# davrempe/contact-human-dynamics

Hardware: NVIDIA H100
Metric: optimised frames/sec (batched phys-optim) (higher is better)
Workload: dtype f64

## Files before the change

__graft_entry__.py:

```python
import os
import subprocess
import sys

ROOT = os.path.dirname(os.path.abspath(__file__))
if ROOT not in sys.path:
    sys.path.insert(0, ROOT)


def build() -> None:
    subprocess.check_call(["make", "-C", os.path.join(ROOT, "contact-human-dynamics_b200", "csrc")])
    subprocess.check_call(["make", "-C", os.path.join(ROOT, "oracle")])
    subprocess.check_call(["make", "-C", os.path.join(ROOT, "tests", "kkt")])
    import chd
    chd.phys.load_lib()


def smoke() -> None:
    import numpy as np
    import chd
    from oracle.phys import OracleProblem
    ps = chd.synth.make_batch(2, 120, 2, seed0=100)
    b = chd.phys.PhysBatch(ps, device=0)
    ev = b.eval("2.2")
    o = OracleProblem(ps[0])
    o.set_stage("2.2")
    n = o.n
    np.testing.assert_allclose(ev["cost"][0], o.cost(), rtol=1e-10)
    np.testing.assert_allclose(ev["grad"][0, :n], o.grad(), rtol=1e-9, atol=1e-9)
    out = b.solve()
    st = out["stage_status"]
    assert (st[[0, 1, 2, 3]] == 0).all() and ((st[4] == 0) | (st[5] == 0)).all(), st
    ref = o.solve()
    ids = {"1.1": 0, "1.2": 1, "2.1": 2, "2.2": 3, "3": 4, "4": 5}
    assert [s["status"] for s in ref["stages"]] == [int(st[ids[k], 0]) for k in ref["stage_ids"]]
    got = out["samples"][2, 0, :out["frames"][0]]
    exp = ref["durations"]
    np.testing.assert_allclose(got[:, :12], exp[:, :12], rtol=0, atol=1e-4)
    np.testing.assert_allclose(got[:, 12:18], exp[:, 12:18], rtol=0, atol=1e-2)
    np.testing.assert_array_equal(got[:, 18:], exp[:, 18:])
    print("smoke ok: launches=%d" % b.launch_count())


if __name__ == "__main__":
    build()
    if len(sys.argv) > 1 and sys.argv[1] == "smoke":
# ... 2 lines not shown
```

contact-human-dynamics_b200/csrc/chd_api.cu:

```cuda
#include <cuda_runtime.h>

#include <cstdio>
#include <cstdlib>
#include <cstring>
#include <vector>

#include "../../include/chd.h"
#include "chd_dev.h"

__global__ void chd_k_stage_begin(ChdDev D);
template <bool GLOBAL>
__global__ void chd_k_eval(ChdDev D);
__global__ void chd_k_init(ChdDev D);
__global__ void chd_k_kkt(ChdDev D);
__global__ void chd_k_kkt_gwin(ChdDev D);
__global__ void chd_k_kcopy(ChdDev D);
__global__ void chd_k_curv(ChdDev D);
__global__ void chd_k_asm(ChdDev D);
__global__ void chd_k_fp64_peak(int mode, int iters, double* sink);
__global__ void chd_k_hess_base(ChdDev D);
__global__ void chd_k_hess_dur(ChdDev D);
__global__ void chd_k_hess_zero(ChdDev D);
__global__ void chd_k_hess_fin(ChdDev D, int mode);
__global__ void chd_k_tables(ChdDev D);
__global__ void chd_k_clear_dyn(ChdDev D);
template <bool GLOBAL>
__global__ void chd_k_linesearch(ChdDev D);
__global__ void chd_k_sample(ChdDev D, double* out, int* frames_out);
__global__ void chd_k_snapshot(ChdDev D, int* frames_out);
__global__ void chd_k_sched_reset(ChdDev D);

#define CHD_CUDA(x)                                                                          \
  do {                                                                                       \
    cudaError_t e_ = (x);                                                                    \
    if (e_ != cudaSuccess) {                                                                 \
      fprintf(stderr, "libchd: CUDA error %s at %s:%d\n", cudaGetErrorString(e_), __FILE__, __LINE__); \
      return -100 - (int)e_;                                                                 \
    }                                                                                        \
  } while (0)

enum { KT_EVAL = 0, KT_KKT = 1, KT_LS = 2, KT_INIT = 3, KT_SAMPLE = 4, KT_N = 8 };

struct ChdIterForm {
  void (*eval)(ChdDev);
  void (*linesearch)(ChdDev);
  size_t smem_eval, smem_ls;
};
static ChdIterForm chd_iter_form(int n_max, int smem_optin) {
  const size_t red = CHD_THREADS * sizeof(double);
  if ((2 * (size_t)n_max + CHD_THREADS) * sizeof(double) + 1024 <= (size_t)smem_optin)
    return {chd_k_eval<false>, chd_k_linesearch<false>, 2 * (size_t)n_max * sizeof(double) + red,
            (size_t)n_max * sizeof(double) + red};
  return {chd_k_eval<true>, chd_k_linesearch<true>, red, red};
}

struct chd_phys_batch {
  ChdHostBatch hb;
  ChdDev D;
  std::vector<void*> allocs;
  cudaStream_t stream = nullptr, copy_stream = nullptr;
  cudaEvent_t ev_kkt = nullptr, ev_ls = nullptr, ev_copy = nullptr;
  int64_t launches = 0;
  int timing = 0;
  bool host_only = false;
  double kt_ms[KT_N] = {0};
  int64_t kt_n[KT_N] = {0};
  cudaEvent_t ev0 = nullptr, ev1 = nullptr;
  int* d_frames = nullptr;
  double* d_samples = nullptr;
  ChdIterForm iter = {};
  size_t smem_kkt = 0;
  int kcopy_blocks = 1;
  ChdIpm* h_ipm = nullptr;
  double* d_x0 = nullptr;
  int64_t h2d_bytes = 0;
  ChdStageDev* d_stages = nullptr;
  int sched_max_iter = 0;
  bool sched_has_dur = false;
  double *poly_T0 = nullptr, *poly_tend0 = nullptr, *phase_tend0 = nullptr;
  int* ent_col0 = nullptr;
};

namespace {

template <class T>
int dev_upload(chd_phys_batch* b, const std::vector<T>& v, const T** out) {
  void* p = nullptr;
  size_t bytes = std::max<size_t>(v.size(), 1) * sizeof(T);
  CHD_CUDA(cudaMallocAsync(&p, bytes, b->stream));
  b->allocs.push_back(p);
  if (!v.empty()) CHD_CUDA(cudaMemcpyAsync(p, v.data(), v.size() * sizeof(T), cudaMemcpyHostToDevice, b->stream));
  b->h2d_bytes += (int64_t)(v.size() * sizeof(T));
  *out = (const T*)p;
  return 0;
}
template <class T>
int dev_alloc(chd_phys_batch* b, size_t count, T** out) {
  void* p = nullptr;
  CHD_CUDA(cudaMallocAsync(&p, std::max<size_t>(count, 1) * sizeof(T), b->stream));
  CHD_CUDA(cudaMemsetAsync(p, 0, std::max<size_t>(count, 1) * sizeof(T), b->stream));
  b->allocs.push_back(p);
  *out = (T*)p;
  return 0;
}
// ... 22 lines not shown
      cudaEventRecord(b->ev1, b->stream);
      cudaEventSynchronize(b->ev1);
      float ms = 0;
      cudaEventElapsedTime(&ms, b->ev0, b->ev1);
      b->kt_ms[id] += ms;
    }
  }
};

void launch_eval(chd_phys_batch* b) {
  Timer t(b, KT_EVAL);
  b->iter.eval<<<b->hb.B, CHD_THREADS, b->iter.smem_eval, b->stream>>>(b->D);
}

int set_schedule(chd_phys_batch* b, const int* sched, int nsched, int override_stage, int override_max_iter) {
  ChdStageDev tab[6];
  for (int s = 0; s < 6; ++s) tab[s] = stage_dev(b->hb.stage[s], s);
  if (override_stage >= 0 && override_max_iter > 0) tab[override_stage].max_iter = override_max_iter;
  CHD_CUDA(cudaMemcpyAsync(b->d_stages, tab, sizeof(tab), cudaMemcpyHostToDevice, b->stream));
  b->D.stages = b->d_stages;
  b->D.nsched = nsched;
  for (int i = 0; i < nsched; ++i) b->D.sched[i] = sched[i];
  b->sched_max_iter = 0;
  b->sched_has_dur = false;
  for (int i = 0; i < nsched; ++i) b->sched_max_iter += tab[sched[i]].max_iter + 2, b->sched_has_dur |= sched[i] == CHD_STAGE_3;
  chd_k_sched_reset<<<(b->hb.B + 127) / 128, 128, 0, b->stream>>>(b->D);
  b->launches++;
  return 0;
}

int run_schedule(chd_phys_batch* b) {
  const int B = b->hb.B;
  const int check_every = 8;
  for (int it = 0; it <= b->sched_max_iter; ++it) {
    {
      Timer t(b, KT_INIT);
      chd_k_stage_begin<<<B, CHD_THREADS, 0, b->stream>>>(b->D);
    }
    launch_eval(b);
    {
      Timer t(b, KT_INIT);
      chd_k_init<<<B, CHD_THREADS, 0, b->stream>>>(b->D);
    }
    {
      Timer t(b, KT_INIT);
      chd_k_hess_zero<<<dim3(8, B), 256, 0, b->stream>>>(b->D);
      chd_k_hess_base<<<dim3(16, B), 256, 0, b->stream>>>(b->D);
      chd_k_hess_fin<<<B, 128, 0, b->stream>>>(b->D, 0);
      b->launches += 2;
    }
    CHD_CUDA(cudaStreamWaitEvent(b->stream, b->ev_copy, 0));
    chd_k_asm<<<dim3(8, B), 256, 0, b->stream>>>(b->D);
    b->launches++;
    {
      Timer t(b, KT_KKT);
      if (b->D.win_smem) chd_k_kkt<<<B, CHD_KKT_THREADS, b->smem_kkt, b->stream>>>(b->D);
      else chd_k_kkt_gwin<<<B, CHD_KKT_THREADS, b->smem_kkt, b->stream>>>(b->D);
    }
    CHD_CUDA(cudaEventRecord(b->ev_kkt, b->stream));
    CHD_CUDA(cudaStreamWaitEvent(b->copy_stream, b->ev_kkt, 0));
    chd_k_kcopy<<<dim3(b->kcopy_blocks, B), 256, 0, b->copy_stream>>>(b->D);
    b->launches++;
    {
      Timer t(b, KT_LS);
      b->iter.linesearch<<<B, CHD_THREADS, b->iter.smem_ls, b->stream>>>(b->D);
    }
    CHD_CUDA(cudaEventRecord(b->ev_ls, b->stream));
    CHD_CUDA(cudaStreamWaitEvent(b->copy_stream, b->ev_ls, 0));
    if (b->sched_has_dur) {
      chd_k_hess_dur<<<dim3(8, B), CHD_THREADS, 0, b->copy_stream>>>(b->D);
      chd_k_hess_fin<<<B, 128, 0, b->copy_stream>>>(b->D, 1);
      b->launches += 2;
    }
    chd_k_curv<<<dim3(8, B), 256, 0, b->copy_stream>>>(b->D);
    b->launches++;
    CHD_CUDA(cudaEventRecord(b->ev_copy, b->copy_stream));
    {
      Timer t(b, KT_SAMPLE);
      chd_k_snapshot<<<B, 128, 0, b->stream>>>(b->D, b->d_frames);
    }
    if ((it % check_every) == check_every - 1) {
      CHD_CUDA(cudaMemcpyAsync(b->h_ipm, b->D.ipm, B * sizeof(ChdIpm), cudaMemcpyDeviceToHost, b->stream));
      CHD_CUDA(cudaStreamSynchronize(b->stream));
      bool any = false;
      for (int i = 0; i < B; ++i) any |= (b->h_ipm[i].phase != CHD_PH_FINISHED);
      if (!any) break;
    }
  }
  CHD_CUDA(cudaMemcpyAsync(b->h_ipm, b->D.ipm, B * sizeof(ChdIpm), cudaMemcpyDeviceToHost, b->stream));
  CHD_CUDA(cudaStreamSynchronize(b->stream));
  CHD_CUDA(cudaStreamSynchronize(b->copy_stream));
  CHD_CUDA(cudaGetLastError());
  return 0;
}

}

extern "C" {

const char* chd_version(void) { return "libchd 0.1 (sm_90a)"; }

int chd_measure_fp64_peak(double* dfma_gflops, double* dmma_gflops) {
  int dev = 0, sms = 0;
  CHD_CUDA(cudaGetDevice(&dev));
  CHD_CUDA(cudaDeviceGetAttribute(&sms, cudaDevAttrMultiProcessorCount, dev));
  double* sink = nullptr;
  CHD_CUDA(cudaMalloc((void**)&sink, sizeof(double) * 1024));
  cudaEvent_t e0, e1;
  CHD_CUDA(cudaEventCreate(&e0));
  CHD_CUDA(cudaEventCreate(&e1));
  const int blocks = sms * 8, threads = 256, iters = 4096;
  for (int mode = 0; mode < 2; ++mode) {
    float best = 1e30f;
    for (int rep = 0; rep < 4; ++rep) {
      CHD_CUDA(cudaEventRecord(e0));
      chd_k_fp64_peak<<<blocks, threads>>>(mode, iters, sink);
      CHD_CUDA(cudaEventRecord(e1));
      CHD_CUDA(cudaEventSynchronize(e1));
      float ms = 0;
// ... 79 lines not shown
  AL(sc, mm) AL(dL, mm) AL(dU, mm) AL(s, mm) AL(y, mm) AL(zL, mm) AL(zU, mm) AL(ds, mm) AL(dy, mm) AL(dzL, mm) AL(dzU, mm)
  int dev = 0, sms = 0, smem_max = 0;
  CHD_CUDA(cudaGetDevice(&dev));
  CHD_CUDA(cudaDeviceGetAttribute(&sms, cudaDevAttrMultiProcessorCount, dev));
  CHD_CUDA(cudaDeviceGetAttribute(&smem_max, cudaDevAttrMaxSharedMemoryPerBlockOptin, dev));
  cudaFuncAttributes fa_kkt, fa_gwin;
  CHD_CUDA(cudaFuncGetAttributes(&fa_kkt, chd_k_kkt));
  CHD_CUDA(cudaFuncGetAttributes(&fa_gwin, chd_k_kkt_gwin));
  const ChdKktPlan P = chd_kkt_plan(hb.Na_max, hb.nb_max, hb.w_max, hb.w_fix_max, hb.n_max, fa_kkt.sharedSizeBytes,
                                    fa_gwin.sharedSizeBytes, (size_t)smem_max);
  D.win_smem = P.win_smem, D.nbc_max = P.nbc_max, D.Q = P.Q, D.Qfix = P.Qfix, D.nbt = P.nbt, D.win_tiles = P.win_tiles;
  D.pan_doubles = P.pan_doubles, D.kstride = P.kstride, D.scratch_stride = P.scratch_stride;
  b->smem_kkt = P.smem_bytes;
  b->kcopy_blocks = (int)std::min<size_t>(512, std::max<size_t>(std::max<size_t>(1, 4 * (size_t)sms / B), P.kstride * sizeof(double) / 131072));
  AL(cost, B * 2) AL(Kwork, B * P.kstride) AL(Kbase, B * P.kstride) AL(sol, B * (size_t)(hb.Na_max + hb.nb_max)) AL(ipm, B)
  AL(rhs0, B * (size_t)(hb.Na_max + hb.nb_max)) AL(rhs1, B * (size_t)(hb.Na_max + hb.nb_max))
  if (P.scratch_stride) AL(scratch, B * P.scratch_stride)
#undef AL
  if ((rc = dev_upload(b, hb.x0, (const double**)&b->d_x0))) return rc;
  CHD_CUDA(cudaMemcpyAsync(D.x, b->d_x0, nm * sizeof(double), cudaMemcpyDeviceToDevice, b->stream));
  b->iter = chd_iter_form(hb.n_max, smem_max);
  if (P.status == CHD_KKT_TOO_WIDE_COMPACT || P.status == CHD_KKT_TOO_WIDE_PAIRS) {
    fprintf(stderr, "libchd: band + border too wide for the %s (Q=%d nbt=%d)\n",
            P.status == CHD_KKT_TOO_WIDE_COMPACT ? "compacted update loop" : "pair tables", P.Q, P.nbt);
    return -5;
  }
  if (P.status == CHD_KKT_TOO_LARGE) {
    fprintf(stderr, "libchd: KKT band + border too large for the shared memory of the factorisation (n_max=%d)\n", hb.n_max);
    return -5;
  }
  CHD_CUDA(cudaFuncSetAttribute(b->iter.eval, cudaFuncAttributeMaxDynamicSharedMemorySize, (int)b->iter.smem_eval));
  CHD_CUDA(cudaFuncSetAttribute(P.win_smem ? chd_k_kkt : chd_k_kkt_gwin, cudaFuncAttributeMaxDynamicSharedMemorySize, (int)b->smem_kkt));
  CHD_CUDA(cudaFuncSetAttribute(b->iter.linesearch, cudaFuncAttributeMaxDynamicSharedMemorySize, (int)b->iter.smem_ls));
  const size_t stride = 6 + 7 * (size_t)hb.n_ee_max;
  CHD_CUDA(cudaMallocAsync((void**)&b->d_samples, B * hb.fo_max * stride * sizeof(double), b->stream));
  CHD_CUDA(cudaMallocAsync((void**)&b->d_frames, B * sizeof(int), b->stream));
  b->allocs.push_back(b->d_samples);
  b->allocs.push_back(b->d_frames);
  b->h_ipm = (ChdIpm*)std::malloc(B * sizeof(ChdIpm));
  if (!b->h_ipm) return -3;
  CHD_CUDA(cudaMallocAsync((void**)&b->d_stages, 6 * sizeof(ChdStageDev), b->stream));
  b->allocs.push_back(b->d_stages);
  if ((rc = dev_alloc(b, 3 * B * hb.fo_max * stride, &D.snapshots))) return rc;
  CHD_CUDA(cudaStreamSynchronize(b->stream));
  return 0;
}

void chd_phys_batch_destroy(chd_phys_batch* b) {
  if (!b) return;
  if (b->stream) {
    for (void* p : b->allocs) cudaFreeAsync(p, b->stream);
    cudaStreamSynchronize(b->stream);
  }
  std::free(b->h_ipm);
  if (b->ev0) cudaEventDestroy(b->ev0);
  if (b->ev1) cudaEventDestroy(b->ev1);
  if (b->ev_kkt) cudaEventDestroy(b->ev_kkt);
  if (b->ev_copy) cudaEventDestroy(b->ev_copy);
  if (b->ev_ls) cudaEventDestroy(b->ev_ls);
  if (b->copy_stream) cudaStreamDestroy(b->copy_stream);
  if (b->stream) cudaStreamDestroy(b->stream);
  delete b;
}

int chd_phys_get_dims(const chd_phys_batch* b, chd_phys_dims* d) {
  if (!b || !d) return -1;
// ... 231 lines not shown
```

contact-human-dynamics_b200/csrc/chd_kkt.cu:

```cuda
#include <cuda_runtime.h>

#include "chd_block.cuh"
#include "chd_eval.cuh"
#include "chd_kkt_tiles.cuh"

__device__ __forceinline__ void chd_hess_sample(const ChdCtx& c, const ChdKT& K, const int* vk, int s, const ChdSpl* P, const double* sign, int np,
                                                int deriv, double wgt, int lane, double* ws) {
  const bool tau = c.opt_dur && s >= 2 && deriv == 0;
  if (lane < 28) {
    const int pa = lane / 14, q = lane % 14;
    double v0 = 0.0, v1 = 0.0, v2 = 0.0;
    int ia = -1;
    if (pa < np) {
      if (q < 12) {
        const int va = P[pa].var[q];
        const double wa = sign[pa] * chd_slot_w(P[pa], deriv, q);
        if (va >= 0 && wa != 0.0) {
          ia = vk[va];
          v0 = q % 3 == 0 ? wa : 0.0, v1 = q % 3 == 1 ? wa : 0.0, v2 = q % 3 == 2 ? wa : 0.0;
        }
      } else if (tau) {
        ChdTau u;
        chd_spl_tau(c, s, s - 2, P[pa], u);
        const int var = q == 12 ? u.va : u.vb;
        const double* dv = q == 12 ? u.da : u.db;
        if (var >= 0) ia = vk[var], v0 = sign[pa] * dv[0], v1 = sign[pa] * dv[1], v2 = sign[pa] * dv[2];
      }
    }
    ws[lane * 4 + 0] = (double)ia, ws[lane * 4 + 1] = v0, ws[lane * 4 + 2] = v1, ws[lane * 4 + 3] = v2;
  }
  __syncwarp();
  const int ne = np * 14;
// ... 274 lines not shown
        if (ka < 0) continue;
        const double va = sc * Jv[ea];
        if (va == 0.0) continue;
        g_add(ka, -va * coef0, va * beta);
        for (int eb = e0; eb < e1; ++eb) {
          const int cb = ec[eb];
          if (cb < 0) continue;
          const int kb = vk[cb];
          if (kb < 0 || ka < kb) continue;
          const double vb = sc * Jv[eb];
          if (vb != 0.0) chd_kadd(K, ka, kb, Sig * va * vb);
        }
      }
    }
  }
}

struct ChdKktCtx {
  int b, tid, nt, lane, warp, nwarp;
  ChdIpm* I;
  ChdStageDev sg;
  const ChdSeq* h;
  int n, m, n_act, Qs, Q, nbt, nbp8, nbl, nbc, NBR, nbt_s;
  size_t ro, vo, n_even, xs_len, win_region;
  const int *rf, *vk, *rk, *ep, *ec;
  const double *Jv, *grad;
  ChdKT K;
  double *red, *cc, *ypan, *xpan, *dinv, *win, *bwin, *vecn, *xs, *xs2;
  double sf, mu, tau, delta_w;
  bool polish;
};

template <bool WS>
__device__ __forceinline__ void chd_kkt_ctx_init(const ChdDev& D, ChdIpm& I, ChdKktCtx& c) {
  extern __shared__ double sm[];
  const int b = blockIdx.x;
  c.b = b, c.I = &I;
  c.sg = D.stages[I.stage];
  const ChdSeq* h = c.h = D.seq + b;
  c.n = h->n, c.m = h->m, c.tid = threadIdx.x, c.nt = blockDim.x;
  c.lane = c.tid & 31, c.warp = c.tid >> 5, c.nwarp = c.nt >> 5;
  c.ro = (size_t)b * D.m_max, c.vo = (size_t)b * D.n_max;
  c.rf = D.rflag + c.ro;
  c.vk = D.var_kkt + c.vo;
  c.rk = D.row_kkt + c.ro;
  c.ep = D.ent_ptr + (size_t)b * (D.m_max + 1);
  c.ec = D.ent_col + (size_t)b * D.slots_max;
  c.Jv = D.Jv + (size_t)b * D.slots_max;
  c.grad = D.grad + c.vo;
  ChdKT& K = c.K;
  chd_kt_init(D, h, D.Kwork + (size_t)b * D.kstride, K);
  K.ovf = &I.band_ovf;
  if (!c.sg.opt_dur) K.q = D.Qfix - 1;
  c.n_act = c.sg.opt_dur ? c.n : c.n - h->n_dur;
  c.Qs = K.Q, c.Q = c.sg.opt_dur ? K.Q : D.Qfix, c.nbt = K.nbt, c.nbp8 = K.nbp8, c.nbl = c.sg.opt_dur ? h->nb : h->nb_fix, c.nbc = K.nbc;
  c.NBR = c.nbl, c.nbt_s = (c.nbl + 1 + 7) >> 3;
  c.n_even = (size_t)((D.n_max + 1) & ~1), c.xs_len = (size_t)(8 * D.nbc_max + c.nbp8);
  double* gs = WS ? nullptr : D.scratch + (size_t)b * D.scratch_stride;
  c.red = sm;
  c.cc = c.red + CHD_KKT_THREADS;
  c.ypan = c.cc + c.nbp8 * c.nbp8;
  c.xpan = c.ypan + (c.Q + c.nbt) * 64;
  c.dinv = c.ypan + D.pan_doubles;
  c.win_region = (size_t)D.win_tiles * 64 + (size_t)c.Qs * c.nbt * 64;
  c.win = WS ? c.dinv + 16 : gs + c.n_even + c.xs_len + 8 * (size_t)D.nbc_max;
  c.bwin = c.win + (size_t)D.win_tiles * 64;
  c.vecn = WS ? c.win + c.win_region - c.n_even : gs;
  c.xs = WS ? c.vecn - c.xs_len : c.vecn + c.n_even;
  c.xs2 = WS ? c.ypan : c.xs + c.xs_len;
  c.sf = I.sf;
}

__device__ __forceinline__ bool chd_kkt_errors(const ChdDev& D, ChdKktCtx& c, int& s_fail) {
  ChdIpm& I = *c.I;
  const int b = c.b, tid = c.tid, nt = c.nt, n = c.n, m = c.m, n_act = c.n_act;
  const size_t ro = c.ro, vo = c.vo;
  const int *rf = c.rf, *vk = c.vk, *ep = c.ep, *ec = c.ec;
  const double *Jv = c.Jv, *grad = c.grad, sf = c.sf;
  double* red = c.red;
  double mu = I.mu;
  const int* erow = D.ent_row + (size_t)b * D.slots_max;
  const int* cptr = D.col_ptr + (size_t)b * (D.n_max + 1);
  const int* cent = D.col_ent + (size_t)b * D.slots_max;
  double* rowv = D.dy + ro;
  double a_ysum = 0, a_zsum = 0, a_cviol = 0, a_theta = 0, a_rs = 0, a_cmax = -INFINITY, a_cmin = INFINITY, a_violu = 0;
  for (int r = tid; r < m; r += nt) {
    const int f = rf[r];
    if (!(f & CHD_ROW_ACTIVE)) {
      rowv[r] = 0.0;
      continue;
    }
    const double sc = D.sc[ro + r], gval = D.g[ro + r], d = sc * gval, y = D.y[ro + r];
    a_ysum += fabs(y);
    a_violu = fmax(a_violu, fmax(D.row_lo[ro + r] - gval, gval - D.row_hi[ro + r]));
    rowv[r] = sc * y;
    const double rp = chd_row_res(f, d, D.dL[ro + r], D.s[ro + r]);
    a_cviol = fmax(a_cviol, fabs(rp));
    a_theta += fabs(rp);
    if (!(f & CHD_ROW_EQ)) {
      const double zL = D.zL[ro + r], zU = D.zU[ro + r];
      const ChdGaps gap = chd_row_gaps(f, D.s[ro + r], D.dL[ro + r], D.dU[ro + r]);
      a_rs = fmax(a_rs, fabs(-y - zL + zU));
      a_zsum += zL + zU;
      if (f & CHD_ROW_HASL) { const double cp = gap.L * zL; a_cmax = fmax(a_cmax, cp); a_cmin = fmin(a_cmin, cp); }
// ... 138 lines not shown
    const unsigned m0 = __ballot_sync(0xffffffffu, act0), m1 = __ballot_sync(0xffffffffu, act1);
    const unsigned below = (1u << lane) - 1u;
    const int n0 = __popc(m0);
    na = n0 + __popc(m1);
    if (act0) cmp[__popc(m0 & below)] = (unsigned char)lane;
    if (act1) cmp[n0 + __popc(m1 & below)] = (unsigned char)g1;
    __syncwarp();
  }
  const int step = c.nwarp - 1;
  const int nb2 = (na + 1) >> 1, nblk = nb2 * (nb2 + 1) / 2;
  for (int p = warp - 1; p < nblk; p += step) {
    const int bi = s_pairs[p] >> 8, bj = s_pairs[p] & 255;
    const int i1 = 2 * bi + 1, j1 = 2 * bj + 1;
    const int gi[2] = {cmp[2 * bi], cmp[i1 & 63]}, gj[2] = {cmp[2 * bj], cmp[j1 & 63]};
    const bool vi[2] = {true, i1 < na}, vj[2] = {true, j1 < na};
    chd_kkt_update_block(c, gi, gj, vi, vj, bi == bj, GB, band_tile, bord_tile);
  }
}

template <class BandTile, class BordTile>
__device__ __forceinline__ void chd_kkt_update_wide(const ChdKktCtx& c, const unsigned short* s_pairs, const int* gnz, int GB, int Gm,
                                                    int tq, const BandTile& band_tile, const BordTile& bord_tile) {
  auto live = [&](int g) { return g < Gm && (g >= GB || g < tq) && gnz[g]; };
  const int nb2 = (Gm + 1) >> 1, nblk = nb2 * (nb2 + 1) / 2;
  for (int p = c.warp - 1; p < nblk; p += c.nwarp - 1) {
    const int bi = s_pairs[p] >> 8, bj = s_pairs[p] & 255;
    const int gi[2] = {2 * bi, 2 * bi + 1}, gj[2] = {2 * bj, 2 * bj + 1};
    const bool vi[2] = {live(gi[0]), live(gi[1])}, vj[2] = {live(gj[0]), live(gj[1])};
    if (!(vi[0] || vi[1]) || !(vj[0] || vj[1])) continue;
    chd_kkt_update_block(c, gi, gj, vi, vj, bi == bj, GB, band_tile, bord_tile);
  }
}

template <bool WS>
__device__ __forceinline__ void chd_kkt_factor(const ChdKktCtx& c, int& s_fail) {
  const ChdKT& K = c.K;
  const int tid = c.tid, nt = c.nt, lane = c.lane, warp = c.warp, nwarp = c.nwarp;
  const int Qs = c.Qs, Q = c.Q, nbt = c.nbt, nbp8 = c.nbp8, nbc = c.nbc, nbt_s = c.nbt_s;
  double *cc = c.cc, *ypan = c.ypan, *xpan = c.xpan, *dinv = c.dinv, *win = c.win, *bwin = c.bwin;
  for (int i = tid; i < nbp8 * nbp8; i += nt) cc[i] = K.corn[i];
  if (WS) {
    for (int idx = tid; idx < Q * Q * 64; idx += nt) {
      const int e = idx & 63, pr = idx >> 6, J = pr / Q, t = pr % Q;
      if (J + t < Q && J < nbc && J + t < nbc) win[chd_win_slot(J + t, J, Q) * 64 + e] = K.band[((size_t)J * Qs + t) * 64 + e];
    }
    for (int idx = tid; idx < Q * nbt * 64; idx += nt) {
      const int J = idx / (nbt * 64);
      if (J < nbc) bwin[idx] = K.bord[(size_t)J * nbt * 64 + idx % (nbt * 64)];
    }
  }
  __syncthreads();
  __shared__ int s_rs[2][96];
  __shared__ int s_gnz[2][96];
  constexpr int kPairs = WS ? 3000 : CHD_KKT_GROUPS_MAX * (CHD_KKT_GROUPS_MAX + 1) / 2;
  __shared__ unsigned short s_pairs[kPairs];
  __shared__ unsigned char s_cmp[CHD_KKT_THREADS / 32][64];
  __shared__ __align__(16) double s_winv[2][64];
#ifdef CHD_PROFILE
  __shared__ unsigned long long s_upd_end;
  double prof_diag = 0.0, prof_upd = 0.0;
  if (tid == 0) s_upd_end = 0;
#endif
  const int GB = K.q, Gm = K.q + nbt_s, nb2 = (Gm + 1) >> 1, npairs = nb2 * (nb2 + 1) / 2;
  for (int p = tid; p < npairs && p < kPairs; p += nt) {
    int gi = (int)((sqrt(8.0 * p + 1.0) - 1.0) * 0.5);
    while (gi * (gi + 1) / 2 > p) --gi;
    while ((gi + 1) * (gi + 2) / 2 <= p) ++gi;
    s_pairs[p] = (unsigned short)((gi << 8) | (p - gi * (gi + 1) / 2));
  }
  auto tri = [](int a_, int b_) { return a_ > b_ ? a_ * (a_ + 1) / 2 + b_ : b_ * (b_ + 1) / 2 + a_; };
  for (int g = tid; g < GB; g += nt) s_rs[0][g] = (1 + g) % Q;
  for (int g = tid; g < 96; g += nt) s_gnz[0][g] = 0, s_gnz[1][g] = 0;
  if (warp == 0) {
    const bool ok = chd_tile_ldl(WS ? win : K.band, dinv, s_winv[0], lane);
    if (!ok && lane == 0) s_fail = 1;
  }
  __syncthreads();
  int kslot = 0, cur = 0;
  for (int Kc = 0; Kc < nbc; ++Kc, cur ^= 1) {
    const int tq = min(K.q, nbc - 1 - Kc);
    const int* rs = s_rs[cur];
    auto band_tile = [&](int gi, int gj) -> double* {
      return WS ? win + (size_t)tri(rs[gi], rs[gj]) * 64 : K.band + ((size_t)(Kc + 1 + gj) * Qs + (gi - gj)) * 64;
    };
    auto bord_tile = [&](int bi, int gj) -> double* {
      return WS ? bwin + ((size_t)rs[gj] * nbt + bi) * 64 : K.bord + ((size_t)(Kc + 1 + gj) * nbt + bi) * 64;
    };
    double* Tkk = WS ? win + (size_t)tri(kslot, kslot) * 64 : K.band + (size_t)Kc * Qs * 64;
    double* Bk = WS ? bwin + (size_t)kslot * nbt * 64 : K.bord + (size_t)Kc * nbt * 64;
    const double* dv = dinv + 8 * cur;
    if (GB == 0 && Kc > 0) {
      if (warp == 0) {
        const bool ok = chd_tile_ldl(Tkk, dinv + 8 * cur, s_winv[cur], lane);
        if (!ok && lane == 0) s_fail = 1;
      }
      __syncthreads();
    }
    {
      const double* wv = s_winv[cur];
      const int r = lane >> 2, k = lane & 3, ng = tq + nbt_s;
      const double2 wf = *reinterpret_cast<const double2*>(wv + 2 * lane);
      const double d0 = dv[2 * k], d1 = dv[2 * k + 1];
      const int f0 = r * 8 + chd_frag_col(2 * k), f1 = r * 8 + chd_frag_col(2 * k + 1);
      for (int g0 = 2 * warp; g0 < ng; g0 += 2 * nwarp) {
        double2 a[2], y[2];
#pragma unroll
        for (int h = 0; h < 2; ++h) {
          const int g = g0 + h;
          const double* A = g < tq ? (WS ? win + (size_t)tri(rs[g], kslot) * 64 : K.band + ((size_t)Kc * Qs + 1 + g) * 64) : Bk + (g - tq) * 64;
          a[h] = g < ng ? make_double2(A[r * 8 + k], A[r * 8 + k + 4]) : make_double2(0.0, 0.0);
          y[h] = make_double2(0.0, 0.0);
        }
        chd_mma_16x8x8(y[0], y[1], a[0], a[1], wf);
#pragma unroll
        for (int h = 0; h < 2; ++h) {
          const int g = g0 + h;
          if (g >= ng) break;
          const bool band_t = g < tq;
          const int pg = band_t ? g : GB + (g - tq);
          const double x0 = y[h].x * d0, x1 = y[h].y * d1;
          ypan[pg * 64 + f0] = y[h].x, ypan[pg * 64 + f1] = y[h].y;
          xpan[pg * 64 + f0] = x0, xpan[pg * 64 + f1] = x1;
          double* G = band_t ? K.band + ((size_t)Kc * Qs + 1 + g) * 64 : K.bord + ((size_t)Kc * nbt + (g - tq)) * 64;
          *reinterpret_cast<double2*>(G + r * 8 + 2 * k) = make_double2(x0, x1);
          const bool nz = __any_sync(0xffffffffu, x0 != 0.0 || x1 != 0.0);
          if (lane == 0 && nz) s_gnz[cur][pg] = 1;
        }
      }
    }
    if (WS)
      for (int e = tid; e < 64; e += nt) K.band[(size_t)Kc * Qs * 64 + e] = Tkk[e];
    __syncthreads();
    const int In = Kc + Q;
#ifdef CHD_PROFILE
    const long long tc0 = clock64();
#endif
    if (WS && In < nbc) {
      for (int idx = tid - 32; idx < Q * 32 + nbt_s * 32; idx += nt - 32) {
        if (idx < 0) break;
        const int tile = idx >> 5, off = (idx & 31) * 2;
        if (tile < Q) {
          const int J = tile < GB ? Kc + 1 + tile : In;
          double* dst = tile < GB ? win + (size_t)tri(kslot, rs[tile]) * 64 : Tkk;
          chd_copy16(dst + off, K.band + ((size_t)J * Qs + (In - J)) * 64 + off, WS);
        } else {
          chd_copy16(Bk + (tile - Q) * 64 + off, K.bord + (size_t)In * nbt * 64 + (tile - Q) * 64 + off, WS);
        }
      }
    }
    if (warp == 0) {
      if (tq >= 1) {
        double* Tn = band_tile(0, 0);
        chd_tile_sub_xyT(Tn, xpan, ypan, lane);
        __syncwarp();
        const bool ok = chd_tile_ldl(Tn, dinv + 8 * (cur ^ 1), s_winv[cur ^ 1], lane);
        if (!ok && lane == 0) s_fail = 1;
      }
#ifdef CHD_PROFILE
      if (lane == 0) prof_diag += (double)(clock64() - tc0);
#endif
    } else {
      if (warp == 1) {
        for (int g = lane; g < GB; g += 32) {
          int v = kslot + 2 + g;
          while (v >= Q) v -= Q;
          s_rs[cur ^ 1][g] = v;
        }
        for (int g = lane; g < Gm; g += 32) s_gnz[cur ^ 1][g] = 0;
      }
      if (!WS && Gm > 64) chd_kkt_update_wide(c, s_pairs, s_gnz[cur], GB, Gm, tq, band_tile, bord_tile);
      else chd_kkt_update_compact(c, s_pairs, s_cmp[warp], s_gnz[cur], GB, Gm, tq, band_tile, bord_tile);
#ifdef CHD_PROFILE
      if (lane == 0) atomicMax(&s_upd_end, (unsigned long long)clock64());
#endif
    }
    chd_copy_wait(WS);
    __syncthreads();
#ifdef CHD_PROFILE
    if (tid == 0) prof_upd += (double)((long long)s_upd_end - tc0);
#endif
    kslot = kslot + 1 == Q ? 0 : kslot + 1;
  }
#ifdef CHD_PROFILE
  if (tid == 0) c.I->prof[6] += prof_diag, c.I->prof[7] += prof_upd;
#endif
}

__device__ __forceinline__ void chd_kkt_border(const ChdDev& D, const ChdKktCtx& c, int& s_fail) {
  const int tid = c.tid, nt = c.nt, lane = c.lane, warp = c.warp, nbl = c.nbl, nbp8 = c.nbp8, NBR = c.NBR, Na = c.K.Na;
  double* cc = c.cc;
  for (int k = 0; k < nbl; ++k) {
    const double dk = cc[k * nbp8 + k];
    if (tid == 0 && !(dk > 0.0 && isfinite(dk))) s_fail = 1;
    __syncthreads();
    const double ik = 1.0 / dk;
    const int rem = nbl - k - 1;
    for (int idx = tid; idx < rem * rem; idx += nt) {
      const int i = k + 1 + idx / rem, j = k + 1 + idx % rem;
      if (j <= i) cc[i * nbp8 + j] -= cc[i * nbp8 + k] * ik * cc[j * nbp8 + k];
    }
    for (int j = k + 1 + tid; j < nbl; j += nt) cc[NBR * nbp8 + j] -= cc[j * nbp8 + k] * ik * cc[NBR * nbp8 + k];
    __syncthreads();
  }
  double* xb = c.xs + 8 * D.nbc_max;
  if (warp == 0) {
    for (int j = lane; j < nbl; j += 32) xb[j] = cc[NBR * nbp8 + j];
    __syncwarp();
    for (int k = nbl - 1; k >= 0; --k) {
      const double xk = xb[k] / cc[k * nbp8 + k];
      __syncwarp();
      for (int j = lane; j < k; j += 32) xb[j] -= cc[k * nbp8 + j] * xk;
      if (lane == 0) xb[k] = xk;
      __syncwarp();
    }
  }
  __syncthreads();
  for (int i = tid; i < nbl; i += nt) D.sol[(size_t)c.b * (D.Na_max + D.nb_max) + Na + i] = xb[i];
}
// ... 233 lines not shown
  ChdKT K;
  chd_kt_init(D, D.seq + b, D.Kwork + (size_t)b * D.kstride, K);
  K.ovf = &D.ipm[b].band_ovf;
  if (!D.stages[I.stage].opt_dur) K.q = D.Qfix - 1;
  const size_t go = (size_t)b * (D.Na_max + D.nb_max);
  chd_assemble(D, b, K, I.delta_w, I.sf, blockIdx.x * blockDim.x + threadIdx.x, gridDim.x * blockDim.x, D.rhs0 + go, D.rhs1 + go);
}

__global__ void __launch_bounds__(256) chd_k_fp64_peak(int mode, int iters, double* sink) {
  const double s = 1.0 + 1e-9 * threadIdx.x;
  double2 a[8];
#pragma unroll
  for (int i = 0; i < 8; ++i) a[i] = make_double2(0.5 + i, 1.5 + i);
  if (mode == 0) {
    for (int it = 0; it < iters; ++it) {
#pragma unroll
      for (int i = 0; i < 8; ++i) a[i].x = fma(a[i].x, s, 1e-3);
    }
  } else {
    const double2 x = make_double2(s, s), y = make_double2(1.0 - 1e-9 * threadIdx.x, 1.0);
    for (int it = 0; it < iters; ++it) {
#pragma unroll
      for (int i = 0; i < 4; ++i) chd_mma_16x8x8(a[2 * i], a[2 * i + 1], x, x, y);
    }
  }
  double t = 0;
#pragma unroll
  for (int i = 0; i < 8; ++i) t += a[i].x + a[i].y;
  if (t == 123.456) sink[threadIdx.x] = t;
}

__global__ void __launch_bounds__(CHD_KKT_THREADS) chd_k_kkt(ChdDev D) { chd_kkt_body<true>(D); }
__global__ void __launch_bounds__(CHD_KKT_THREADS) chd_k_kkt_gwin(ChdDev D) { chd_kkt_body<false>(D); }
```

contact-human-dynamics_b200/csrc/chd_kkt_plan.h:

```cpp
#pragma once
#include <cstddef>

#include "chd_core.h"

#define CHD_KKT_THREADS 512
#define CHD_KKT_GROUPS_MAX 96
#define CHD_SMEM_OPTIN 232448
#define CHD_KKT_GWIN_STATIC_MAX 16384

enum ChdKktStatus {
  CHD_KKT_FITS = 0,
  CHD_KKT_TOO_WIDE_COMPACT = 1,
  CHD_KKT_TOO_WIDE_PAIRS = 2,
  CHD_KKT_TOO_LARGE = 3,
};

CHD_HD size_t chd_kkt_gwin_smem(int Q, int nbt) {
  return (CHD_KKT_THREADS + 64 * (size_t)nbt * nbt + 2 * (size_t)(Q + nbt) * 64 + 16) * sizeof(double);
}
CHD_HD int chd_kkt_gwin_status(int w_max, int nb_max, size_t gwin_static, size_t smem_optin) {
  const int Q = (w_max + 7) / 8 + 1, nbt = (nb_max + 1 + 7) / 8;
  if (Q - 1 + nbt > CHD_KKT_GROUPS_MAX) return CHD_KKT_TOO_WIDE_PAIRS;
  if (chd_kkt_gwin_smem(Q, nbt) + gwin_static + 256 > smem_optin) return CHD_KKT_TOO_LARGE;
  return CHD_KKT_FITS;
}

struct ChdKktPlan {
  int status;
  int win_smem;
  int nbc_max, Q, Qfix, nbt;
  int win_tiles, pan_doubles;
  size_t kstride;
  size_t smem_bytes;
  size_t scratch_stride;
};

CHD_HD ChdKktPlan chd_kkt_plan(int Na_max, int nb_max, int w_max, int w_fix_max, int n_max, size_t kkt_static,
                               size_t gwin_static, size_t smem_optin) {
// ... 27 lines not shown
```

Before: 13700.

## Split KKT block factorization across a 2-CTA cluster with DSMEM ring

Adds a cluster-launched KKT kernel in which CTA 0 factors the band while CTA 1 processes the border columns. Panels are streamed to CTA 1 through a distributed-shared-memory ring guarded by mbarriers, and CTA 1 copies the corner block back at the end. The host tracks how many problems are still live and uses the cluster path only when that count fits the occupancy-reported cluster capacity. This aims to cut per-problem KKT latency when few problems remain, at the cost of doubling the CTAs per problem and adding cross-CTA synchronisation.

```diff
diff --git a/__graft_entry__.py b/__graft_entry__.py
--- a/__graft_entry__.py
+++ b/__graft_entry__.py
@@ -11,6 +11,7 @@
     subprocess.check_call(["make", "-C", os.path.join(ROOT, "contact-human-dynamics_b200", "csrc")])
     subprocess.check_call(["make", "-C", os.path.join(ROOT, "oracle")])
     subprocess.check_call(["make", "-C", os.path.join(ROOT, "tests", "kkt")])
+    subprocess.check_call(["make", "-C", os.path.join(ROOT, "tests", "kkt_cluster")])
     import chd
     chd.phys.load_lib()
 
diff --git a/contact-human-dynamics_b200/csrc/chd_api.cu b/contact-human-dynamics_b200/csrc/chd_api.cu
--- a/contact-human-dynamics_b200/csrc/chd_api.cu
+++ b/contact-human-dynamics_b200/csrc/chd_api.cu
@@ -14,6 +14,7 @@
 __global__ void chd_k_init(ChdDev D);
 __global__ void chd_k_kkt(ChdDev D);
 __global__ void chd_k_kkt_gwin(ChdDev D);
+__global__ void chd_k_kkt_cl(ChdDev D, int ring_max);
 __global__ void chd_k_kcopy(ChdDev D);
 __global__ void chd_k_curv(ChdDev D);
 __global__ void chd_k_asm(ChdDev D);
@@ -70,6 +71,7 @@
   double* d_samples = nullptr;
   ChdIterForm iter = {};
   size_t smem_kkt = 0;
+  int kkt_clusters = 0;
   int kcopy_blocks = 1;
   ChdIpm* h_ipm = nullptr;
   double* d_x0 = nullptr;
@@ -158,6 +160,7 @@
 int run_schedule(chd_phys_batch* b) {
   const int B = b->hb.B;
   const int check_every = 8;
+  int live = B;
   for (int it = 0; it <= b->sched_max_iter; ++it) {
     {
       Timer t(b, KT_INIT);
@@ -180,8 +183,19 @@
     b->launches++;
     {
       Timer t(b, KT_KKT);
-      if (b->D.win_smem) chd_k_kkt<<<B, CHD_KKT_THREADS, b->smem_kkt, b->stream>>>(b->D);
-      else chd_k_kkt_gwin<<<B, CHD_KKT_THREADS, b->smem_kkt, b->stream>>>(b->D);
+      if (b->D.win_smem && live <= b->kkt_clusters) {
+        cudaLaunchConfig_t cfg = {};
+        cudaLaunchAttribute attr[1];
+        attr[0].id = cudaLaunchAttributeClusterDimension;
+        attr[0].val.clusterDim.x = 2, attr[0].val.clusterDim.y = 1, attr[0].val.clusterDim.z = 1;
+        cfg.gridDim = dim3(2 * B), cfg.blockDim = dim3(CHD_KKT_THREADS), cfg.dynamicSmemBytes = b->smem_kkt;
+        cfg.stream = b->stream, cfg.attrs = attr, cfg.numAttrs = 1;
+        CHD_CUDA(cudaLaunchKernelEx(&cfg, chd_k_kkt_cl, b->D, (int)CHD_KKT_RING));
+      } else if (b->D.win_smem) {
+        chd_k_kkt<<<B, CHD_KKT_THREADS, b->smem_kkt, b->stream>>>(b->D);
+      } else {
+        chd_k_kkt_gwin<<<B, CHD_KKT_THREADS, b->smem_kkt, b->stream>>>(b->D);
+      }
     }
     CHD_CUDA(cudaEventRecord(b->ev_kkt, b->stream));
     CHD_CUDA(cudaStreamWaitEvent(b->copy_stream, b->ev_kkt, 0));
@@ -208,9 +222,9 @@
     if ((it % check_every) == check_every - 1) {
       CHD_CUDA(cudaMemcpyAsync(b->h_ipm, b->D.ipm, B * sizeof(ChdIpm), cudaMemcpyDeviceToHost, b->stream));
       CHD_CUDA(cudaStreamSynchronize(b->stream));
-      bool any = false;
-      for (int i = 0; i < B; ++i) any |= (b->h_ipm[i].phase != CHD_PH_FINISHED);
-      if (!any) break;
+      live = 0;
+      for (int i = 0; i < B; ++i) live += b->h_ipm[i].phase != CHD_PH_FINISHED;
+      if (!live) break;
     }
   }
   CHD_CUDA(cudaMemcpyAsync(b->h_ipm, b->D.ipm, B * sizeof(ChdIpm), cudaMemcpyDeviceToHost, b->stream));
@@ -356,6 +370,19 @@
   CHD_CUDA(cudaFuncSetAttribute(b->iter.eval, cudaFuncAttributeMaxDynamicSharedMemorySize, (int)b->iter.smem_eval));
   CHD_CUDA(cudaFuncSetAttribute(P.win_smem ? chd_k_kkt : chd_k_kkt_gwin, cudaFuncAttributeMaxDynamicSharedMemorySize, (int)b->smem_kkt));
   CHD_CUDA(cudaFuncSetAttribute(b->iter.linesearch, cudaFuncAttributeMaxDynamicSharedMemorySize, (int)b->iter.smem_ls));
+  if (P.win_smem) {
+    cudaLaunchConfig_t cfg = {};
+    cudaLaunchAttribute attr[1];
+    attr[0].id = cudaLaunchAttributeClusterDimension;
+    attr[0].val.clusterDim.x = 2, attr[0].val.clusterDim.y = 1, attr[0].val.clusterDim.z = 1;
+    cfg.gridDim = dim3(2 * B), cfg.blockDim = dim3(CHD_KKT_THREADS), cfg.dynamicSmemBytes = b->smem_kkt;
+    cfg.attrs = attr, cfg.numAttrs = 1;
+    if (cudaFuncSetAttribute(chd_k_kkt_cl, cudaFuncAttributeMaxDynamicSharedMemorySize, (int)b->smem_kkt) != cudaSuccess ||
+        cudaOccupancyMaxActiveClusters(&b->kkt_clusters, chd_k_kkt_cl, &cfg) != cudaSuccess) {
+      b->kkt_clusters = 0;
+      cudaGetLastError();
+    }
+  }
   const size_t stride = 6 + 7 * (size_t)hb.n_ee_max;
   CHD_CUDA(cudaMallocAsync((void**)&b->d_samples, B * hb.fo_max * stride * sizeof(double), b->stream));
   CHD_CUDA(cudaMallocAsync((void**)&b->d_frames, B * sizeof(int), b->stream));
diff --git a/contact-human-dynamics_b200/csrc/chd_kkt.cu b/contact-human-dynamics_b200/csrc/chd_kkt.cu
--- a/contact-human-dynamics_b200/csrc/chd_kkt.cu
+++ b/contact-human-dynamics_b200/csrc/chd_kkt.cu
@@ -1,3 +1,4 @@
+#include <cooperative_groups.h>
 #include <cuda_runtime.h>
 
 #include "chd_block.cuh"
@@ -338,9 +339,8 @@
 };
 
 template <bool WS>
-__device__ __forceinline__ void chd_kkt_ctx_init(const ChdDev& D, ChdIpm& I, ChdKktCtx& c) {
+__device__ __forceinline__ void chd_kkt_ctx_init(const ChdDev& D, ChdIpm& I, ChdKktCtx& c, int b) {
   extern __shared__ double sm[];
-  const int b = blockIdx.x;
   c.b = b, c.I = &I;
   c.sg = D.stages[I.stage];
   const ChdSeq* h = c.h = D.seq + b;
@@ -376,6 +376,10 @@
   c.xs2 = WS ? c.ypan : c.xs + c.xs_len;
   c.sf = I.sf;
 }
+template <bool WS>
+__device__ __forceinline__ void chd_kkt_ctx_init(const ChdDev& D, ChdIpm& I, ChdKktCtx& c) {
+  chd_kkt_ctx_init<WS>(D, I, c, blockIdx.x);
+}
 
 __device__ __forceinline__ bool chd_kkt_errors(const ChdDev& D, ChdKktCtx& c, int& s_fail) {
   ChdIpm& I = *c.I;
@@ -580,19 +584,53 @@
   }
 }
 
-template <bool WS>
+struct ChdKktRing {
+  unsigned base;
+  int dlog;
+};
+__shared__ unsigned long long chd_kkt_ring_full[CHD_KKT_RING], chd_kkt_ring_empty[CHD_KKT_RING];
+__shared__ ChdKktRing chd_kkt_ring;
+__device__ __forceinline__ int chd_kkt_ring_slot_doubles(int Qs, int nbt) { return (Qs - 1 + nbt) * 64 + 64 + 8 + 32; }
+__device__ __forceinline__ void chd_st_cluster(unsigned addr, double v) {
+  asm volatile("st.shared::cluster.f64 [%0], %1;" ::"r"(addr), "d"(v) : "memory");
+}
+__device__ __forceinline__ void chd_st_cluster(unsigned addr, double2 v) {
+  asm volatile("st.shared::cluster.v2.f64 [%0], {%1, %2};" ::"r"(addr), "d"(v.x), "d"(v.y) : "memory");
+}
+__device__ __forceinline__ void chd_st_cluster(unsigned addr, int v) {
+  asm volatile("st.shared::cluster.u32 [%0], %1;" ::"r"(addr), "r"(v) : "memory");
+}
+__device__ __forceinline__ void chd_mbar_init(unsigned long long* bar, unsigned count) {
+  asm volatile("mbarrier.init.shared::cta.b64 [%0], %1;" ::"r"((unsigned)__cvta_generic_to_shared(bar)), "r"(count) : "memory");
+}
+__device__ __forceinline__ void chd_mbar_arrive_cluster(unsigned long long* bar, unsigned rank) {
+  unsigned ra;
+  asm volatile("mapa.shared::cluster.u32 %0, %1, %2;" : "=r"(ra) : "r"((unsigned)__cvta_generic_to_shared(bar)), "r"(rank));
+  asm volatile("mbarrier.arrive.release.cluster.shared::cluster.b64 _, [%0];" ::"r"(ra) : "memory");
+}
+__device__ __forceinline__ void chd_mbar_wait(unsigned long long* bar, unsigned parity) {
+  const unsigned a = (unsigned)__cvta_generic_to_shared(bar);
+  unsigned ok;
+  do {
+    asm volatile("{\n .reg .pred p;\n mbarrier.try_wait.parity.acquire.cluster.shared::cta.b64 p, [%1], %2;\n selp.u32 %0, 1, 0, p;\n}"
+                 : "=r"(ok) : "r"(a), "r"(parity) : "memory");
+  } while (!ok);
+}
+
+template <bool WS, bool CL = false>
 __device__ __forceinline__ void chd_kkt_factor(const ChdKktCtx& c, int& s_fail) {
   const ChdKT& K = c.K;
   const int tid = c.tid, nt = c.nt, lane = c.lane, warp = c.warp, nwarp = c.nwarp;
   const int Qs = c.Qs, Q = c.Q, nbt = c.nbt, nbp8 = c.nbp8, nbc = c.nbc, nbt_s = c.nbt_s;
   double *cc = c.cc, *ypan = c.ypan, *xpan = c.xpan, *dinv = c.dinv, *win = c.win, *bwin = c.bwin;
-  for (int i = tid; i < nbp8 * nbp8; i += nt) cc[i] = K.corn[i];
+  if (!CL)
+    for (int i = tid; i < nbp8 * nbp8; i += nt) cc[i] = K.corn[i];
   if (WS) {
     for (int idx = tid; idx < Q * Q * 64; idx += nt) {
       const int e = idx & 63, pr = idx >> 6, J = pr / Q, t = pr % Q;
       if (J + t < Q && J < nbc && J + t < nbc) win[chd_win_slot(J + t, J, Q) * 64 + e] = K.band[((size_t)J * Qs + t) * 64 + e];
     }
-    for (int idx = tid; idx < Q * nbt * 64; idx += nt) {
+    for (int idx = tid; idx < (CL ? 0 : Q * nbt * 64); idx += nt) {
       const int J = idx / (nbt * 64);
       if (J < nbc) bwin[idx] = K.bord[(size_t)J * nbt * 64 + idx % (nbt * 64)];
     }
@@ -610,6 +648,7 @@
   if (tid == 0) s_upd_end = 0;
 #endif
   const int GB = K.q, Gm = K.q + nbt_s, nb2 = (Gm + 1) >> 1, npairs = nb2 * (nb2 + 1) / 2;
+  const int Gu = CL ? GB : Gm;
   for (int p = tid; p < npairs && p < kPairs; p += nt) {
     int gi = (int)((sqrt(8.0 * p + 1.0) - 1.0) * 0.5);
     while (gi * (gi + 1) / 2 > p) --gi;
@@ -646,7 +685,7 @@
     }
     {
       const double* wv = s_winv[cur];
-      const int r = lane >> 2, k = lane & 3, ng = tq + nbt_s;
+      const int r = lane >> 2, k = lane & 3, ng = CL ? tq : tq + nbt_s;
       const double2 wf = *reinterpret_cast<const double2*>(wv + 2 * lane);
       const double d0 = dv[2 * k], d1 = dv[2 * k + 1];
       const int f0 = r * 8 + chd_frag_col(2 * k), f1 = r * 8 + chd_frag_col(2 * k + 1);
@@ -684,7 +723,7 @@
     const long long tc0 = clock64();
 #endif
     if (WS && In < nbc) {
-      for (int idx = tid - 32; idx < Q * 32 + nbt_s * 32; idx += nt - 32) {
+      for (int idx = tid - 32; idx < Q * 32 + (CL ? 0 : nbt_s * 32); idx += nt - 32) {
         if (idx < 0) break;
         const int tile = idx >> 5, off = (idx & 31) * 2;
         if (tile < Q) {
@@ -716,11 +755,29 @@
         }
         for (int g = lane; g < Gm; g += 32) s_gnz[cur ^ 1][g] = 0;
       }
+      if (CL) {
+        const ChdKktRing ring = chd_kkt_ring;
+        const int rsd = chd_kkt_ring_slot_doubles(Qs, nbt);
+        const unsigned rY = ring.base + (unsigned)((Kc & ((1 << ring.dlog) - 1)) * rsd) * 8u;
+        for (int i = tid - 32; i < tq * 32; i += nt - 32) chd_st_cluster(rY + i * 16, reinterpret_cast<const double2*>(ypan)[i]);
+        if (warp == nwarp - 1) {
+          const unsigned rW = rY + (rsd - 104) * 8;
+          chd_st_cluster(rW + lane * 16, reinterpret_cast<const double2*>(s_winv[cur])[lane]);
+          if (lane < 4) chd_st_cluster(rW + 512 + lane * 16, reinterpret_cast<const double2*>(dv)[lane]);
+          for (int g = lane; g < tq; g += 32) chd_st_cluster(rW + 576 + g * 4, s_gnz[cur][g]);
+        }
+        __syncwarp();
+        if (lane == 0) chd_mbar_arrive_cluster(chd_kkt_ring_full + (Kc & ((1 << ring.dlog) - 1)), 1);
+      }
       if (!WS && Gm > 64) chd_kkt_update_wide(c, s_pairs, s_gnz[cur], GB, Gm, tq, band_tile, bord_tile);
-      else chd_kkt_update_compact(c, s_pairs, s_cmp[warp], s_gnz[cur], GB, Gm, tq, band_tile, bord_tile);
+      else chd_kkt_update_compact(c, s_pairs, s_cmp[warp], s_gnz[cur], GB, Gu, tq, band_tile, bord_tile);
 #ifdef CHD_PROFILE
       if (lane == 0) atomicMax(&s_upd_end, (unsigned long long)clock64());
 #endif
+      if (CL && tid == nt - 1) {
+        const int dl = chd_kkt_ring.dlog;
+        if (Kc + 1 >= (1 << dl)) chd_mbar_wait(chd_kkt_ring_empty + ((Kc + 1) & ((1 << dl) - 1)), ((Kc + 1 >> dl) - 1) & 1);
+      }
     }
     chd_copy_wait(WS);
     __syncthreads();
@@ -732,6 +789,117 @@
 #ifdef CHD_PROFILE
   if (tid == 0) c.I->prof[6] += prof_diag, c.I->prof[7] += prof_upd;
 #endif
+}
+
+__device__ __forceinline__ void chd_kkt_factor_border(const ChdKktCtx& c) {
+  const ChdKktRing ring = chd_kkt_ring;
+  const ChdKT& K = c.K;
+  const int tid = c.tid, nt = c.nt, lane = c.lane, warp = c.warp, nwarp = c.nwarp;
+  const int Q = c.Q, nbt = c.nbt, nbp8 = c.nbp8, nbc = c.nbc, nbt_s = c.nbt_s, GB = K.q;
+  double *cc = c.cc, *bwin = c.bwin;
+  unsigned char* cmp = reinterpret_cast<unsigned char*>(c.red) + warp * 64;
+  int* bgnz = reinterpret_cast<int*>(c.red + 128);
+  unsigned short* cpairs = reinterpret_cast<unsigned short*>(c.red + 160);
+  const int rbm = (nbt_s + 1) >> 1;
+  for (int p = tid; p < rbm * (rbm + 1) / 2; p += nt) {
+    int i = 0;
+    while ((i + 1) * (i + 2) / 2 <= p) ++i;
+    cpairs[p] = (unsigned short)((i << 8) | (p - i * (i + 1) / 2));
+  }
+  for (int i = tid; i < nbp8 * nbp8; i += nt) cc[i] = K.corn[i];
+  for (int idx = tid; idx < Q * nbt * 64; idx += nt) {
+    const int J = idx / (nbt * 64);
+    if (J < nbc) bwin[idx] = K.bord[(size_t)J * nbt * 64 + idx % (nbt * 64)];
+  }
+  __syncthreads();
+  ChdKktCtx cb = c;
+  cb.xpan = bwin - (size_t)(GB + nbt) * 64;
+  auto band_tile = [](int, int) -> double* { return nullptr; };
+  const int rsd = chd_kkt_ring_slot_doubles(c.Qs, nbt);
+  int kslot = 0;
+  for (int Kc = 0; Kc < nbc; ++Kc) {
+    const int tq = min(GB, nbc - 1 - Kc);
+    const int rslot = Kc & ((1 << ring.dlog) - 1), ruse = Kc >> ring.dlog;
+    double* S = c.ypan + (size_t)rslot * rsd;
+    const double* wv = S + rsd - 104;
+    const double* dv = wv + 64;
+    const int* gz = reinterpret_cast<const int*>(dv + 8);
+    double* Bk = bwin + (size_t)kslot * nbt * 64;
+    cb.ypan = S;
+    chd_mbar_wait(chd_kkt_ring_full + rslot, ruse & 1);
+    {
+      const int r = lane >> 2, k = lane & 3;
+      const double2 wf = *reinterpret_cast<const double2*>(wv + 2 * lane);
+      const double d0 = dv[2 * k], d1 = dv[2 * k + 1];
+      const int f0 = r * 8 + chd_frag_col(2 * k), f1 = r * 8 + chd_frag_col(2 * k + 1);
+      for (int g0 = 2 * warp; g0 < nbt_s; g0 += 2 * nwarp) {
+        double2 a[2], y[2];
+#pragma unroll
+        for (int h = 0; h < 2; ++h) {
+          const double* A = Bk + (g0 + h) * 64;
+          a[h] = g0 + h < nbt_s ? make_double2(A[r * 8 + k], A[r * 8 + k + 4]) : make_double2(0.0, 0.0);
+          y[h] = make_double2(0.0, 0.0);
+        }
+        chd_mma_16x8x8(y[0], y[1], a[0], a[1], wf);
+#pragma unroll
+        for (int h = 0; h < 2; ++h) {
+          const int g = g0 + h, pg = GB + g;
+          if (g >= nbt_s) break;
+          const double x0 = y[h].x * d0, x1 = y[h].y * d1;
+          S[pg * 64 + f0] = y[h].x, S[pg * 64 + f1] = y[h].y;
+          cb.xpan[pg * 64 + f0] = x0, cb.xpan[pg * 64 + f1] = x1;
+          *reinterpret_cast<double2*>(K.bord + ((size_t)Kc * nbt + g) * 64 + r * 8 + 2 * k) = make_double2(x0, x1);
+          const bool nz = __any_sync(0xffffffffu, x0 != 0.0 || x1 != 0.0);
+          if (lane == 0) bgnz[g] = nz;
+        }
+      }
+    }
+    __syncthreads();
+    const int In = Kc + Q;
+    if (In < nbc)
+      for (int idx = tid; idx < nbt_s * 32; idx += nt)
+        chd_copy16(Bk + (idx >> 5) * 64 + (idx & 31) * 2, K.bord + (size_t)In * nbt * 64 + (idx >> 5) * 64 + (idx & 31) * 2, 1);
+    auto bord_tile = [&](int bi, int gj) -> double* {
+      int v = kslot + 1 + gj;
+      if (v >= Q) v -= Q;
+      return bwin + ((size_t)v * nbt + bi) * 64;
+    };
+    int nbd, nbr;
+    {
+      const bool a0 = lane < tq && gz[lane], a1 = lane + 32 < tq && gz[lane + 32];
+      const bool b0 = lane < nbt_s && bgnz[lane], b1 = lane + 32 < nbt_s && bgnz[lane + 32];
+      const unsigned ma0 = __ballot_sync(0xffffffffu, a0), ma1 = __ballot_sync(0xffffffffu, a1);
+      const unsigned mb0 = __ballot_sync(0xffffffffu, b0), mb1 = __ballot_sync(0xffffffffu, b1);
+      const unsigned below = (1u << lane) - 1u;
+      nbd = __popc(ma0) + __popc(ma1);
+      nbr = __popc(mb0) + __popc(mb1);
+      if (a0) cmp[__popc(ma0 & below)] = (unsigned char)lane;
+      if (a1) cmp[__popc(ma0) + __popc(ma1 & below)] = (unsigned char)(lane + 32);
+      if (b0) cmp[nbd + __popc(mb0 & below)] = (unsigned char)(GB + lane);
+      if (b1) cmp[nbd + __popc(mb0) + __popc(mb1 & below)] = (unsigned char)(GB + lane + 32);
+      __syncwarp();
+    }
+    const int rb = (nbr + 1) >> 1, cbd = (nbd + 1) >> 1, nbb = rb * cbd, nblk = nbb + rb * (rb + 1) / 2;
+    const unsigned char* rowl = cmp + nbd;
+    for (int p = warp; p < nblk; p += nwarp) {
+      int bi, bj;
+      const unsigned char* coll;
+      int ncol;
+      if (p < nbb) {
+        bi = p / cbd, bj = p - bi * cbd, coll = cmp, ncol = nbd;
+      } else {
+        bi = cpairs[p - nbb] >> 8, bj = cpairs[p - nbb] & 255, coll = rowl, ncol = nbr;
+      }
+      const int i1 = 2 * bi + 1, j1 = 2 * bj + 1;
+      const int gi[2] = {rowl[2 * bi], rowl[i1 < nbr ? i1 : 2 * bi]}, gj[2] = {coll[2 * bj], coll[j1 < ncol ? j1 : 2 * bj]};
+      const bool vi[2] = {true, i1 < nbr}, vj[2] = {true, j1 < ncol};
+      chd_kkt_update_block(cb, gi, gj, vi, vj, p >= nbb && bi == bj, GB, band_tile, bord_tile);
+    }
+    chd_copy_wait(1);
+    __syncthreads();
+    if (tid == 0) chd_mbar_arrive_cluster(chd_kkt_ring_empty + rslot, 0);
+    kslot = kslot + 1 == Q ? 0 : kslot + 1;
+  }
 }
 
 __device__ __forceinline__ void chd_kkt_border(const ChdDev& D, const ChdKktCtx& c, int& s_fail) {
@@ -1031,3 +1199,59 @@
 
 __global__ void __launch_bounds__(CHD_KKT_THREADS) chd_k_kkt(ChdDev D) { chd_kkt_body<true>(D); }
 __global__ void __launch_bounds__(CHD_KKT_THREADS) chd_k_kkt_gwin(ChdDev D) { chd_kkt_body<false>(D); }
+
+namespace cg = cooperative_groups;
+template <class Before, class After>
+__device__ __forceinline__ void chd_kkt_cl_body(const ChdDev& D, int ring_max, const Before& before_factor, const After& after_factor) {
+  __shared__ int s_fail, s_go;
+  cg::cluster_group cluster = cg::this_cluster();
+  const unsigned rank = cluster.block_rank();
+  const int b = blockIdx.x >> 1;
+  ChdIpm& I = D.ipm[b];
+  if (I.phase != CHD_PH_RUN) return;
+  ChdKktCtx c;
+  chd_kkt_ctx_init<true>(D, I, c, b);
+  if (c.tid == 0) {
+    ChdKktRing ring;
+    const int fit = (int)((size_t)(c.bwin - c.ypan - c.nbt * 64) / chd_kkt_ring_slot_doubles(c.Qs, c.nbt));
+    const int depth = min(min(ring_max, CHD_KKT_RING), fit);
+    ring.dlog = depth >= 4 ? 2 : (depth >= 2 ? 1 : 0);
+    const unsigned a = (unsigned)__cvta_generic_to_shared(c.ypan);
+    if (rank) ring.base = a;
+    else asm("mapa.shared::cluster.u32 %0, %1, 1;" : "=r"(ring.base) : "r"(a));
+    for (int i = 0; i < (1 << ring.dlog); ++i) chd_mbar_init((rank ? chd_kkt_ring_full : chd_kkt_ring_empty) + i, rank ? c.nwarp - 1 : 1);
+    chd_kkt_ring = ring;
+  }
+  asm volatile("fence.mbarrier_init.release.cluster;" ::: "memory");
+  cluster.sync();
+  if (rank == 0) {
+    const bool done = before_factor(c, s_fail);
+    if (c.tid == 0) *cluster.map_shared_rank(&s_go, 1) = !done;
+    cluster.sync();
+    if (done) return;
+    chd_kkt_factor<true, true>(c, s_fail);
+    cluster.sync();
+    after_factor(c, s_fail);
+  } else {
+    cluster.sync();
+    if (!s_go) return;
+    chd_kkt_factor_border(c);
+    double2* dst = reinterpret_cast<double2*>(cluster.map_shared_rank(c.cc, 0));
+    for (int i = c.tid; i < c.nbp8 * c.nbp8 / 2; i += c.nt) dst[i] = reinterpret_cast<const double2*>(c.cc)[i];
+    cluster.sync();
+  }
+}
+__global__ void __launch_bounds__(CHD_KKT_THREADS) chd_k_kkt_cl(ChdDev D, int ring_max) {
+  auto before = [&](ChdKktCtx& c, int& s_fail) {
+    if (chd_kkt_errors(D, c, s_fail)) return true;
+    chd_kkt_assemble(D, c);
+    return false;
+  };
+  chd_kkt_cl_body(D, ring_max, before, [&](const ChdKktCtx& c, int& s_fail) {
+    chd_kkt_border(D, c, s_fail);
+    chd_kkt_backsub<true>(D, c);
+    if (chd_kkt_no_step(D, c, s_fail)) return;
+    __syncthreads();
+    chd_kkt_recover(D, c);
+  });
+}
diff --git a/contact-human-dynamics_b200/csrc/chd_kkt_plan.h b/contact-human-dynamics_b200/csrc/chd_kkt_plan.h
--- a/contact-human-dynamics_b200/csrc/chd_kkt_plan.h
+++ b/contact-human-dynamics_b200/csrc/chd_kkt_plan.h
@@ -4,6 +4,7 @@
 #include "chd_core.h"
 
 #define CHD_KKT_THREADS 512
+#define CHD_KKT_RING 4
 #define CHD_KKT_GROUPS_MAX 96
 #define CHD_SMEM_OPTIN 232448
 #define CHD_KKT_GWIN_STATIC_MAX 16384
```

Measured after the change: 13930 (median of 6 runs). +1.7%, better.
